# tgp-team/torch-geometric-pool

Hardware: NVIDIA B200
Metric: coarsened graphs/s (Reduce+Connect fwd+bwd) (higher is better)
Workload: dtype f32

## Files before the change

torch-geometric-pool_b200/csrc/dense_bwd_fused.cu:

```cuda
#include <stdlib.h>
#include <string.h>

#include "dense.cuh"
#include "tc_gemm.cuh"
#include "tc_ptx.cuh"

namespace tgp {
namespace tc {

extern long long* g_engine_dbg;

namespace {

#ifndef TGPB200_BWD_EPI_WARPS
#define TGPB200_BWD_EPI_WARPS 4
#endif
#ifndef TGPB200_ABL
#define TGPB200_ABL 0
#endif
#ifndef TGPB200_BWD_CONCAT
#define TGPB200_BWD_CONCAT 0
#endif
constexpr bool kConcat = TGPB200_BWD_CONCAT != 0;
constexpr int kPairs = 7;
constexpr int kGroups = 2;
constexpr int kSlots = kConcat ? 2 : 4;
static_assert(kSlots % kGroups == 0, "every operand slot must belong to ONE split group (its waiters see every phase)");
constexpr int kEpiW = TGPB200_BWD_EPI_WARPS;
constexpr int kThreadsBwd = 64 + kGroups * 128 + kEpiW * 32;
constexpr int BK = 32, KSTEPS = 4;
constexpr int BNB = 64;
constexpr uint32_t kAccW = kConcat ? 128 : 64;
constexpr uint32_t kColW = 0, kColS = kAccW, kColX = 2 * kAccW, kColRing = 2 * kAccW + 128, kRing = 64;
static_assert(kColRing + kSlots * kRing <= 512, "tensor memory budget");
constexpr uint32_t kABytes = BM * kStageRowBytes, kBBytes = BNB * kStageRowBytes;
constexpr uint32_t kStage = kABytes + 2 * kBBytes;
constexpr uint32_t kEpiBufs = kEpiW == 4 ? 2 : 1;
constexpr uint32_t kEpiBytes = kEpiW * kEpiBufs * 4096;
constexpr uint32_t kHookBytes = BM * BNB * 4;

enum ASrc { kAKMajor = 0, kAMnPlain = 1, kATmem = 2 };

struct BwdParams {
  CUtensorMap map_a[kPairs], map_b[kPairs];
  int kd[kPairs], a_src[kPairs], b_mn[kPairs], b_n0[kPairs], first[kPairs], wide[kPairs];
  uint32_t acc_col[kPairs];
  int num_pairs;
  int batch, N, K, F;
  int m_tiles, num_items, stages;
  CUtensorMap map_ds, map_dx;
  const float* S;
  const float* d;
  const float* coef;
  const float* uv;
  float eps;
  long long* dbg;
};

__global__ void __launch_bounds__(kThreadsBwd, 1) k_dense_bwd_fused(const __grid_constant__ BwdParams P) {
  extern __shared__ __align__(1024) uint8_t smem_raw[];
  uint8_t* smem = reinterpret_cast<uint8_t*>((reinterpret_cast<uintptr_t>(smem_raw) + 1023) & ~(uintptr_t)1023);
  const int stages = P.stages;
  uint64_t* bars = reinterpret_cast<uint64_t*>(smem + (size_t)kStage * stages + kEpiBytes + kHookBytes);
  const uint32_t bar_base = smem_u32(bars);
  auto bar_full = [&](int s) { return bar_base + 8u * s; };
  auto bar_lo = [&](int s) { return bar_base + 8u * (stages + s); };
  auto bar_empty = [&](int s) { return bar_base + 8u * (2 * stages + s); };
  auto bar_tfree = [&](int g) { return bar_base + 8u * (3 * stages + g); };
  const uint32_t bar_wfull = bar_base + 8u * (3 * stages + kSlots), bar_tfull = bar_wfull + 8u, bar_tempty = bar_wfull + 16u;
  uint32_t* tmem_slot = reinterpret_cast<uint32_t*>(bars + 3 * stages + kSlots + 3);

  const int warp = threadIdx.x >> 5, lane = threadIdx.x & 31;
  const uint32_t smem_base = smem_u32(smem);
  if (P.dbg && threadIdx.x == 0) {
    unsigned long long t;
    uint32_t smid;
    asm volatile("mov.u64 %0, %%globaltimer;" : "=l"(t));
    asm volatile("mov.u32 %0, %%smid;" : "=r"(smid));
    P.dbg[(200 + blockIdx.x) * 8 + 0] = (long long)t;
    P.dbg[(200 + blockIdx.x) * 8 + 2] = (long long)smid;
  }

  if (warp == 0 && lane == 0) {
    for (int s = 0; s < stages; ++s) {
      mbar_init(bar_full(s), 1);
      mbar_init(bar_lo(s), 4);
      mbar_init(bar_empty(s), 1);
    }
    for (int g = 0; g < kSlots; ++g) mbar_init(bar_tfree(g), 1);
    mbar_init(bar_wfull, 1);
    mbar_init(bar_tfull, 1);
    mbar_init(bar_tempty, kEpiW);
    fence_barrier_init();
  }
  if (warp == 1) tmem_alloc(smem_u32(tmem_slot), 512);
  tc_fence_before();
  __syncthreads();
  tc_fence_after();
  const uint32_t tmem_base = *tmem_slot;


  if (warp == 0) {
    int s = 0;
    uint32_t ph = 0;
    for (int item = blockIdx.x; item < P.num_items; item += gridDim.x) {
      const int mt = item % P.m_tiles, b = item / P.m_tiles;
      const int m0 = mt * BM;
      for (int p = 0; p < P.num_pairs; ++p) {
        const int src = P.a_src[p];
        for (int kb = 0, nkb = (P.kd[p] + BK - 1) / BK; kb < nkb; ++kb) {
          mbar_wait(bar_empty(s), ph ^ 1);
          const uint32_t sa = smem_base + (uint32_t)s * kStage, sb = sa + kABytes;
          const int k0 = kb * BK;
          if ((TGPB200_ABL & 64) && elect_one()) mbar_arrive(bar_full(s));
          if (!(TGPB200_ABL & 64) && elect_one()) {
            const bool load_a = src != kATmem && !(TGPB200_ABL & 32);
            mbar_arrive_expect_tx(bar_full(s), (load_a ? kABytes : 0u) + kBBytes);
            if (!load_a) {
            } else if (src == kAMnPlain) tma_load_3d(sa, &P.map_a[p], bar_full(s), m0, k0, b);
            else if (src == kAKMajor) tma_load_3d(sa, &P.map_a[p], bar_full(s), k0, m0, b);
            if (P.b_mn[p]) {
              for (int blk = 0; blk < BNB / 32; ++blk)
                tma_load_3d(sb + blk * (BK * kStageRowBytes), &P.map_b[p], bar_full(s), P.b_n0[p] + blk * 32, k0, b);
            } else {
              tma_load_3d(sb, &P.map_b[p], bar_full(s), k0, P.b_n0[p], b);
            }
          }
          __syncwarp();
          if (++s == stages) { s = 0; ph ^= 1; }
        }
      }
    }
  } else if (warp == 1) {
    const uint32_t tm = __shfl_sync(kFull, tmem_base, 0);
    if (elect_one()) {
      int s = 0;
      uint32_t ph = 0, kc = 0;
      int it = 0;
      for (int item = blockIdx.x; item < P.num_items; item += gridDim.x, ++it) {
        for (int p = 0; p < P.num_pairs; ++p) {
          if (p == 1) {
            mbar_wait(bar_tempty, ((uint32_t)it & 1u) ^ 1u);
            tc_fence_after();
          }
          const uint32_t d_tmem = tm + P.acc_col[p];
          const uint32_t idesc = (1u << 4) | (2u << 7) | (2u << 10) | ((uint32_t)P.b_mn[p] << 16) |
                                 ((uint32_t)(BNB >> 3) << 17) | ((uint32_t)(BM >> 4) << 24);
          const uint32_t b_lbo = P.b_mn[p] ? BK * kStageRowBytes : 16;
          const uint32_t b_step = P.b_mn[p] ? 8 * kStageRowBytes : 32;
          const uint64_t desc_b0 = make_desc(smem_base, b_lbo, P.b_mn[p] ? 512 : 1024, P.b_mn[p] ? 1 : 2);
          const uint32_t idesc2 = (idesc & ~(0x3fu << 17)) | ((uint32_t)((2 * BNB) >> 3) << 17);
          const bool wide = kConcat && P.wide[p] != 0;
          uint32_t accum = P.first[p] ? 0u : 1u;
          for (int kb = 0, nkb = (P.kd[p] + BK - 1) / BK; kb < nkb; ++kb, ++kc) {
            if (P.dbg && blockIdx.x == 0 && kc < 128) P.dbg[kc * 8 + 7] = clock64();
            mbar_wait(bar_lo(s), ph);
            if (P.dbg && blockIdx.x == 0 && kc < 128) P.dbg[kc * 8 + 5] = clock64();
            if (!(TGPB200_ABL & 1024)) tc_fence_after();
            const uint32_t ts = kc % (uint32_t)kSlots;
            const uint32_t a_stage = tm + kColRing + ts * kRing;
            const uint64_t db0 = desc_b0 + (uint64_t)(((uint32_t)s * kStage + kABytes) >> 4);
#pragma unroll
            for (int kk = 0; kk < ((TGPB200_ABL & 128) ? 0 : KSTEPS); ++kk) {
              const uint64_t db = db0 + (uint64_t)(kk * (b_step >> 4)), db_lo = db + (kBBytes >> 4);
              const uint32_t a_hi = a_stage + (uint32_t)(kk * 16), a_lo = a_hi + 8;
              if (wide) {
                umma_ts_tf32(d_tmem, a_hi, db, idesc2, kk == 0 ? accum : 1u);
                umma_ts_tf32(d_tmem, a_lo, db, idesc, 1u);
              } else {
                umma_ts_tf32(d_tmem, a_lo, db, idesc, kk == 0 ? accum : 1u);
                umma_ts_tf32(d_tmem, a_hi, db_lo, idesc, 1u);
                umma_ts_tf32(d_tmem, a_hi, db, idesc, 1u);
              }
            }
            if (P.dbg && blockIdx.x == 0 && kc < 128) P.dbg[kc * 8 + 0] = clock64();
            if (TGPB200_ABL & 4096) mbar_arrive(bar_empty(s)); else umma_commit(bar_empty(s));
            if (TGPB200_ABL & 8192) mbar_arrive(bar_tfree(ts)); else umma_commit(bar_tfree(ts));
            if (P.dbg && blockIdx.x == 0 && kc < 128) P.dbg[kc * 8 + 6] = clock64();
            accum = 1;
            if (++s == stages) { s = 0; ph ^= 1; }
          }
          if (p == 0) umma_commit(bar_wfull);
        }
        umma_commit(bar_tfull);
      }
    }
    __syncwarp();
  } else if (warp < 2 + kGroups * 4) {
    const int grp = (warp - 2) >> 2;
    const int t = (threadIdx.x - 64) & 127;
    const int q = warp & 3;
    const int m_local = q * 32 + lane;
    int s = 0;
    uint32_t ph = 0, kc = 0;
    int it = 0;
    for (int item = blockIdx.x; item < P.num_items; item += gridDim.x, ++it) {
      for (int p = 0; p < P.num_pairs; ++p) {
        const int src = P.a_src[p];
        for (int kb = 0, nkb = (P.kd[p] + BK - 1) / BK; kb < nkb; ++kb, ++kc) {
          if ((int)(kc % (uint32_t)kGroups) != grp) {
            mbar_wait(bar_full(s), ph);
            if (++s == stages) { s = 0; ph ^= 1; }
            continue;
          }
          mbar_wait(bar_full(s), ph);
          const uint32_t sa = smem_base + (uint32_t)s * kStage, sb = sa + kABytes;
          for (uint32_t ch = t; ch < ((TGPB200_ABL & 1) ? 0u : kBBytes / 16); ch += 128) {
            const float4 v = lds128(sb + ch * 16);
            float4 h, l;
            h.x = rna_tf32(v.x), h.y = rna_tf32(v.y), h.z = rna_tf32(v.z), h.w = rna_tf32(v.w);
            l.x = v.x - h.x, l.y = v.y - h.y, l.z = v.z - h.z, l.w = v.w - h.w;
            sts128(sb + ch * 16, h);
            sts128(sb + kBBytes + ch * 16, l);
          }
          if (!(TGPB200_ABL & 2)) fence_proxy_async();
          float x[32];
          if (TGPB200_ABL & 4) {
#pragma unroll
            for (int k = 0; k < 32; ++k) x[k] = (float)(k + lane);
          } else if (src == kATmem) {
            mbar_wait(bar_wfull, (uint32_t)it & 1u);
            tc_fence_after();
            tmem_ld32(tmem_base + ((uint32_t)(q * 32) << 16) + kColW + (uint32_t)(kb * BK), x);
            if (kConcat) {
              float x2[32];
              tmem_ld32(tmem_base + ((uint32_t)(q * 32) << 16) + kColW + 64u + (uint32_t)(kb * BK), x2);
#pragma unroll
              for (int k = 0; k < 32; ++k) x[k] += x2[k];
            }
          } else if (src == kAMnPlain) {
#pragma unroll
            for (int k = 0; k < 32; ++k) x[k] = lds32(sa + (uint32_t)k * (BM * 4) + (uint32_t)m_local * 4);
          } else {
#pragma unroll
            for (int c = 0; c < 8; ++c) {
              const float4 v = lds128(sa + (uint32_t)m_local * kStageRowBytes + (uint32_t)((c ^ (m_local & 7)) << 4));
              x[4 * c] = v.x, x[4 * c + 1] = v.y, x[4 * c + 2] = v.z, x[4 * c + 3] = v.w;
            }
          }
          const uint32_t slot = kc % (uint32_t)kSlots;
          if (TGPB200_ABL & 16384) {
            __syncwarp();
            if (lane == 0) mbar_arrive(bar_lo(s));
            if (++s == stages) { s = 0; ph ^= 1; }
            continue;
          }
          mbar_wait(bar_tfree(slot), ((kc / (uint32_t)kSlots) & 1u) ^ 1u);
          tc_fence_after();
          const uint32_t a_stage = tmem_base + ((uint32_t)(q * 32) << 16) + kColRing + slot * kRing;
#pragma unroll
          for (int kk = 0; kk < KSTEPS; ++kk) {
            float hi[8], lo[8];
#pragma unroll
            for (int i = 0; i < 8; ++i) {
              hi[i] = rna_tf32(x[kk * 8 + i]);
              lo[i] = x[kk * 8 + i] - hi[i];
            }
            if (!(TGPB200_ABL & 8)) tmem_st16(a_stage + (uint32_t)(kk * 16), hi, lo);
            else if (hi[0] == 123.456f && lo[7] == 3.f) P.dbg[0] = 1;
          }
          tmem_st_wait();
          tc_fence_before();
          __syncwarp();
          if (lane == 0) mbar_arrive(bar_lo(s));
          if (P.dbg && blockIdx.x == 0 && lane == 0 && kc < 128) P.dbg[kc * 8 + 1 + q] = clock64();
          if (++s == stages) { s = 0; ph ^= 1; }
        }
      }
    }
  } else {
    const int quad = warp & 3;
    const int ew = warp - 2 - kGroups * 4;
    const int e2 = ew >> 2;
    const uint32_t stg0 = smem_base + (uint32_t)kStage * stages + (uint32_t)ew * kEpiBufs * 4096u;
    uint32_t n_stored = 0;
    const uint32_t hook0 = smem_base + (uint32_t)kStage * stages + kEpiBytes;
    const int n_chunks = 2 + (P.F + 31) / 32;
    int it = 0;
    for (int item = blockIdx.x; item < P.num_items; item += gridDim.x, ++it) {
      const int mt = item % P.m_tiles, b = item / P.m_tiles;
      const int m_base = mt * BM + quad * 32;
      const int m = m_base + lane;
      float dd = 0.f, c_ent = 0.f, di = 0.f;
      bool hook = false;
      const uint32_t hrow = hook0 + (uint32_t)(quad * 32 + lane) * (BNB * 4);
      if (!(TGPB200_ABL & 256) && P.S != nullptr && m < P.N) {
        const float c_den = P.coef[b * 4 + 0];
        c_ent = P.coef[b * 4 + 2];
        hook = c_den != 0.f || c_ent != 0.f;
        if (hook) {
          dd = 2.f * c_den * P.d[(int64_t)b * P.N + m];
          const float* srow = P.S + ((int64_t)b * P.N + m) * P.K;
          for (int j = 0; j * 4 < P.K; ++j) cp_async16(hrow + (uint32_t)((j ^ (lane & 7)) << 4), srow + j * 4);
        }
        if (P.uv != nullptr) di = P.d[(int64_t)b * P.N + m];
      }
      cp_async_commit();
      mbar_wait(bar_tfull, (uint32_t)it & 1u);
      if (P.dbg && blockIdx.x == 0 && ew == 0 && lane == 0 && it < 32) P.dbg[(128 + it) * 8 + 0] = clock64();
      tc_fence_after();
      cp_async_wait_all();
      __syncwarp();
      for (int c = 0; c < ((TGPB200_ABL & 16) ? 0 : n_chunks); ++c) {
        if (kEpiW == 8 && (c & 1) != e2) continue;
        const bool is_ds = c < 2;
        const int n0 = is_ds ? c * 32 : (c - 2) * 32;
        float v[32];
        tmem_ld32(tmem_base + ((uint32_t)(quad * 32) << 16) + (is_ds ? kColS : kColX) + (uint32_t)n0, v);
        if (kConcat && is_ds) {
          float v2[32];
          tmem_ld32(tmem_base + ((uint32_t)(quad * 32) << 16) + kColS + 64u + (uint32_t)n0, v2);
#pragma unroll
          for (int j = 0; j < 32; ++j) v[j] += v2[j];
        }
        if (m_base >= P.N || n0 >= (is_ds ? P.K : P.F)) continue;
        if (is_ds && hook) {
#pragma unroll
          for (int c4 = 0; c4 < 8; ++c4) {
            if (n0 + c4 * 4 < P.K) {
              const float4 t4 = lds128(hrow + (uint32_t)((((n0 >> 2) + c4) ^ (lane & 7)) << 4));
              const float sv[4] = {t4.x, t4.y, t4.z, t4.w};
#pragma unroll
              for (int j = 0; j < 4; ++j) {
                float add = dd * sv[j];
                if (c_ent != 0.f) add += c_ent * (-__logf(sv[j] + P.eps) - __fdividef(sv[j], sv[j] + P.eps));
                v[c4 * 4 + j] += add;
              }
            }
          }
        }
        if (is_ds && P.uv != nullptr) {
          const float* ub = P.uv + (int64_t)b * 2 * P.K + n0;
#pragma unroll
          for (int j = 0; j < 32; ++j)
            if (n0 + j < P.K) v[j] += fmaf(di, __ldg(ub + j), __ldg(ub + P.K + j));
        }
        const uint32_t stg = stg0 + (n_stored % kEpiBufs) * 4096u;
        ++n_stored;
        if (lane == 0) {
          if (kEpiBufs == 2) tma_store_wait_read<1>();
          else tma_store_wait_read<0>();
        }
        __syncwarp();
        const uint32_t row = stg + (uint32_t)lane * 128u;
#pragma unroll
        for (int c4 = 0; c4 < 8; ++c4)
          sts128(row + (uint32_t)((c4 ^ (lane & 7)) << 4), make_float4(v[4 * c4], v[4 * c4 + 1], v[4 * c4 + 2], v[4 * c4 + 3]));
        fence_proxy_async();
        __syncwarp();
        if (lane == 0 && !(TGPB200_ABL & 512)) {
          tma_store_3d(is_ds ? &P.map_ds : &P.map_dx, stg, n0, m_base, b);
          tma_store_commit();
        }
      }
      tc_fence_before();
      __syncwarp();
      if (lane == 0) mbar_arrive(bar_tempty);
      if (P.dbg && blockIdx.x == 0 && ew == 0 && lane == 0 && it < 32) P.dbg[(128 + it) * 8 + 1] = clock64();
    }
    if (lane == 0) tma_store_wait_all();
  }

  tc_fence_before();
  __syncthreads();
  if (P.dbg && threadIdx.x == 0) {
    unsigned long long t;
    asm volatile("mov.u64 %0, %%globaltimer;" : "=l"(t));
    P.dbg[(200 + blockIdx.x) * 8 + 1] = (long long)t;
  }
  if (warp == 1) tmem_dealloc(tmem_base, 512);
}

bool make_out_map(CUtensorMap* map, float* ptr, int64_t batch, int64_t rows, int64_t cols) {
  EncodeTiledFn fn = encode_fn();
  if (!fn || ((uintptr_t)ptr & 15) || (cols % 4)) return false;
  cuuint64_t dims[3] = {(cuuint64_t)cols, (cuuint64_t)rows, (cuuint64_t)batch};
  cuuint64_t strides[2] = {(cuuint64_t)cols * 4, (cuuint64_t)rows * cols * 4};
  cuuint32_t box[3] = {32, 32, 1}, estr[3] = {1, 1, 1};
  return fn(map, CU_TENSOR_MAP_DATA_TYPE_FLOAT32, 3, ptr, dims, strides, box, estr, CU_TENSOR_MAP_INTERLEAVE_NONE,
            CU_TENSOR_MAP_SWIZZLE_128B, CU_TENSOR_MAP_L2_PROMOTION_NONE, CU_TENSOR_MAP_FLOAT_OOB_FILL_NONE) == CUDA_SUCCESS;
}

}

int dense_bwd_fused(const float* A, const float* S, const float* X, const float* Tt, const float* Gx, const float* Graw,
                    const float* Pm, int B, int N, int K, int F, const float* ew_S, const float* ew_d, const float* ew_coef,
                    const float* ew_uv, float eps, float* dS, float* dX, cudaStream_t stream) {
  {
    const char* e = getenv("TGPB200_BWD_FUSED");
    if (e && e[0] == '0') return TGPB200_ERR_UNSUPPORTED;
  }
  if (!A || !S || !X || !Tt || !Gx || !Graw || !dS || !dX || B <= 0) return TGPB200_ERR_UNSUPPORTED;
  if (K > BNB || F > 128 || (N % 4) || (K % 4) || (F % 4) || N < 1) return TGPB200_ERR_UNSUPPORTED;
  const uintptr_t al = (uintptr_t)A | (uintptr_t)S | (uintptr_t)X | (uintptr_t)Tt | (uintptr_t)Gx | (uintptr_t)Graw |
                       (uintptr_t)(Pm ? Pm : Graw);
  if (al & 15) return TGPB200_ERR_UNSUPPORTED;
  BwdParams P;
  memset(&P, 0, sizeof(P));
  P.batch = B, P.N = N, P.K = K, P.F = F;
  P.m_tiles = (N + BM - 1) / BM;
  P.num_items = B * P.m_tiles;
  const int64_t NN = (int64_t)N * N, NK = (int64_t)N * K, NF = (int64_t)N * F, KK = (int64_t)K * K, KF = (int64_t)K * F;
  int n = 0;
  bool ok = true;
  auto add = [&](int kd, int a_src, OperandDesc a, OperandDesc b, int b_n0, uint32_t acc, int first) {
    P.kd[n] = kd, P.a_src[n] = a_src, P.b_mn[n] = b.mn_major, P.b_n0[n] = b_n0, P.acc_col[n] = acc, P.first[n] = first;
    P.wide[n] = acc != kColX && acc != kColX + (uint32_t)BNB;
    if (a_src == kAKMajor) ok = ok && make_operand_map(&P.map_a[n], a, false, B, N, kd, BM);
    else if (a_src == kAMnPlain) ok = ok && make_operand_map_mn_plain(&P.map_a[n], a, B, N, kd);
    ok = ok && make_operand_map(&P.map_b[n], b, false, B, b.mn_major ? (int)b.row_stride : (int)(b.batch_stride / b.row_stride), kd, BNB);
    ++n;
  };
  add(N, kAKMajor, OperandDesc{A, NN, N, 0}, OperandDesc{S, NK, K, 1}, 0, kColW, 1);
  add(F, kAKMajor, OperandDesc{X, NF, F, 0}, OperandDesc{Gx, KF, F, 0}, 0, kColS, 1);
  add(K, kAMnPlain, OperandDesc{Tt, NK, N, 1}, OperandDesc{Graw, KK, K, 1}, 0, kColS, 0);
  if (Pm) add(K, kAKMajor, OperandDesc{S, NK, K, 0}, OperandDesc{Pm, KK, K, 1}, 0, kColS, 0);
  add(K, kATmem, OperandDesc{nullptr, 0, 0, 0}, OperandDesc{Graw, KK, K, 0}, 0, kColS, 0);
  for (int j = 0; j * BNB < F; ++j)
    add(K, kAKMajor, OperandDesc{S, NK, K, 0}, OperandDesc{Gx, KF, F, 1}, j * BNB, kColX + (uint32_t)(j * BNB), 1);
  if (!ok) return TGPB200_ERR_UNSUPPORTED;
  P.num_pairs = n;
  if (!make_out_map(&P.map_ds, dS, B, N, K) || !make_out_map(&P.map_dx, dX, B, N, F)) return TGPB200_ERR_UNSUPPORTED;
  P.S = ew_S, P.d = ew_d, P.coef = ew_coef, P.uv = ew_S ? ew_uv : nullptr, P.eps = eps;
  P.stages = 5;
  {
    const char* e = getenv("TGPB200_BWD_STAGES");
    if (e && atoi(e) >= 2 && atoi(e) <= 5) P.stages = atoi(e);
  }
  P.dbg = g_engine_dbg;
  static bool attr_set = false;
  if (!attr_set) {
    attr_set = true;
    cudaFuncSetAttribute(k_dense_bwd_fused, cudaFuncAttributeMaxDynamicSharedMemorySize, 227 * 1024);
  }
  const size_t smem = (size_t)kStage * P.stages + kEpiBytes + kHookBytes + (3 * P.stages + kSlots + 4) * 8 + 16 + 1024;
  const int sms = device_sm_count();
  const int grid = P.num_items < sms ? P.num_items : sms;
  launch("k_dense_bwd_fused", k_dense_bwd_fused, grid, kThreadsBwd, smem, stream, P);
  return launch_status();
}

}
}
```

torch-geometric-pool_b200/csrc/tc_ptx.cuh:

```cuda
#pragma once
#include <cuda.h>
#include <stdio.h>

#include "common.cuh"

namespace tgp {
namespace tc {

__device__ __forceinline__ uint32_t smem_u32(const void* p) { return (uint32_t)__cvta_generic_to_shared(p); }

__device__ __forceinline__ void mbar_init(uint32_t bar, uint32_t count) {
  asm volatile("mbarrier.init.shared::cta.b64 [%0], %1;" ::"r"(bar), "r"(count));
}
__device__ __forceinline__ void mbar_arrive(uint32_t bar) {
  asm volatile("mbarrier.arrive.shared::cta.b64 _, [%0];" ::"r"(bar) : "memory");
}
__device__ __forceinline__ void mbar_arrive_expect_tx(uint32_t bar, uint32_t bytes) {
  asm volatile("mbarrier.arrive.expect_tx.shared::cta.b64 _, [%0], %1;" ::"r"(bar), "r"(bytes) : "memory");
}
__device__ __forceinline__ void mbar_wait(uint32_t bar, uint32_t parity) {
  uint32_t done = 0;
  uint64_t spins = 0;
  while (true) {
    asm volatile(
        "{\n"
        ".reg .pred p;\n"
        "mbarrier.try_wait.parity.shared::cta.b64 p, [%1], %2;\n"
        "selp.u32 %0, 1, 0, p;\n"
        "}\n"
        : "=r"(done)
        : "r"(bar), "r"(parity)
        : "memory");
    if (done) break;
    if (++spins > (1ull << 26)) {
      printf("[tgp_b200] mbarrier wait timed out (block %d thread %d bar %u parity %u)\n", blockIdx.x, threadIdx.x, bar,
             parity);
      __trap();
    }
  }
}
__device__ __forceinline__ bool elect_one() {
  uint32_t pred;
  asm volatile("{\n.reg .pred p;\nelect.sync _|p, 0xffffffff;\nselp.u32 %0, 1, 0, p;\n}\n" : "=r"(pred));
  return pred != 0;
}
__device__ __forceinline__ void fence_barrier_init() { asm volatile("fence.mbarrier_init.release.cluster;" ::: "memory"); }
__device__ __forceinline__ void fence_proxy_async() { asm volatile("fence.proxy.async.shared::cta;" ::: "memory"); }
__device__ __forceinline__ void tc_fence_before() { asm volatile("tcgen05.fence::before_thread_sync;" ::: "memory"); }
__device__ __forceinline__ void tc_fence_after() { asm volatile("tcgen05.fence::after_thread_sync;" ::: "memory"); }

__device__ __forceinline__ void tma_load_3d(uint32_t dst, const CUtensorMap* map, uint32_t bar, int c0, int c1, int c2) {
  asm volatile(
      "cp.async.bulk.tensor.3d.shared::cluster.global.mbarrier::complete_tx::bytes [%0], [%1, {%3, %4, %5}], [%2];" ::"r"(dst),
      "l"(map), "r"(bar), "r"(c0), "r"(c1), "r"(c2)
      : "memory");
}
__device__ __forceinline__ void tma_load_4d(uint32_t dst, const CUtensorMap* map, uint32_t bar, int c0, int c1, int c2,
                                            int c3) {
  asm volatile(
      "cp.async.bulk.tensor.4d.shared::cluster.global.mbarrier::complete_tx::bytes [%0], [%1, {%3, %4, %5, %6}], [%2];" ::"r"(
          dst),
      "l"(map), "r"(bar), "r"(c0), "r"(c1), "r"(c2), "r"(c3)
      : "memory");
}

__device__ __forceinline__ void tma_store_3d(const CUtensorMap* map, uint32_t src, int c0, int c1, int c2) {
  asm volatile("cp.async.bulk.tensor.3d.global.shared::cta.bulk_group [%0, {%2, %3, %4}], [%1];" ::"l"(map), "r"(src),
               "r"(c0), "r"(c1), "r"(c2)
               : "memory");
}
__device__ __forceinline__ void tma_store_commit() { asm volatile("cp.async.bulk.commit_group;" ::: "memory"); }
template <int kPending>
__device__ __forceinline__ void tma_store_wait_read() {
  asm volatile("cp.async.bulk.wait_group.read %0;" ::"n"(kPending) : "memory");
}
__device__ __forceinline__ void tma_store_wait_all() { asm volatile("cp.async.bulk.wait_group 0;" ::: "memory"); }
__device__ __forceinline__ void cp_async16(uint32_t dst, const void* src) {
  asm volatile("cp.async.cg.shared.global [%0], [%1], 16;" ::"r"(dst), "l"(src) : "memory");
}
__device__ __forceinline__ void cp_async_commit() { asm volatile("cp.async.commit_group;" ::: "memory"); }
__device__ __forceinline__ void cp_async_wait_all() { asm volatile("cp.async.wait_group 0;" ::: "memory"); }
__device__ __forceinline__ void sts32(uint32_t addr, uint32_t v) {
  asm volatile("st.shared.u32 [%0], %1;" ::"r"(addr), "r"(v) : "memory");
}
__device__ __forceinline__ void sts128u(uint32_t addr, const uint4& v) {
  asm volatile("st.shared.v4.u32 [%0], {%1, %2, %3, %4};" ::"r"(addr), "r"(v.x), "r"(v.y), "r"(v.z), "r"(v.w) : "memory");
}

__device__ __forceinline__ void tmem_alloc(uint32_t dst_smem, uint32_t ncols) {
  asm volatile("tcgen05.alloc.cta_group::1.sync.aligned.shared::cta.b32 [%0], %1;" ::"r"(dst_smem), "r"(ncols) : "memory");
  asm volatile("tcgen05.relinquish_alloc_permit.cta_group::1.sync.aligned;" ::: "memory");
}
__device__ __forceinline__ void tmem_dealloc(uint32_t addr, uint32_t ncols) {
  asm volatile("tcgen05.dealloc.cta_group::1.sync.aligned.b32 %0, %1;" ::"r"(addr), "r"(ncols) : "memory");
}
__device__ __forceinline__ void umma_commit(uint32_t bar) {
  asm volatile("tcgen05.commit.cta_group::1.mbarrier::arrive::one.shared::cluster.b64 [%0];" ::"r"(bar) : "memory");
}
template <bool kTf32>
__device__ __forceinline__ void umma(uint32_t tmem_d, uint64_t desc_a, uint64_t desc_b, uint32_t idesc, uint32_t accum) {
  if (kTf32) {
    asm volatile(
        "{\n.reg .pred p;\nsetp.ne.b32 p, %4, 0;\n"
        "tcgen05.mma.cta_group::1.kind::tf32 [%0], %1, %2, %3, p;\n}\n" ::"r"(tmem_d),
        "l"(desc_a), "l"(desc_b), "r"(idesc), "r"(accum)
        : "memory");
  } else {
    asm volatile(
        "{\n.reg .pred p;\nsetp.ne.b32 p, %4, 0;\n"
        "tcgen05.mma.cta_group::1.kind::f16 [%0], %1, %2, %3, p;\n}\n" ::"r"(tmem_d),
        "l"(desc_a), "l"(desc_b), "r"(idesc), "r"(accum)
        : "memory");
  }
}
__device__ __forceinline__ uint32_t cluster_ctarank() {
  uint32_t r;
  asm volatile("mov.u32 %0, %%cluster_ctarank;" : "=r"(r));
  return r;
}
__device__ __forceinline__ uint32_t mapa_shared(uint32_t addr, uint32_t rank) {
  uint32_t r;
  asm volatile("mapa.shared::cluster.u32 %0, %1, %2;" : "=r"(r) : "r"(addr), "r"(rank));
  return r;
}
__device__ __forceinline__ void cluster_sync_all() {
  asm volatile("barrier.cluster.arrive.release.aligned;" ::: "memory");
  asm volatile("barrier.cluster.wait.acquire.aligned;" ::: "memory");
}
__device__ __forceinline__ void mbar_arrive_cluster(uint32_t cluster_bar) {
  asm volatile("mbarrier.arrive.release.cluster.shared::cluster.b64 _, [%0];" ::"r"(cluster_bar) : "memory");
}
__device__ __forceinline__ void tma_load_3d_pair(uint32_t dst, const CUtensorMap* map, uint32_t leader_bar, int c0, int c1,
                                                 int c2) {
  asm volatile(
      "cp.async.bulk.tensor.3d.cta_group::2.shared::cluster.global.mbarrier::complete_tx::bytes [%0], [%1, {%3, %4, %5}], [%2];" ::
          "r"(dst),
      "l"(map), "r"(leader_bar), "r"(c0), "r"(c1), "r"(c2)
      : "memory");
}
__device__ __forceinline__ void tmem_alloc_pair(uint32_t dst_smem, uint32_t ncols) {
  asm volatile("tcgen05.alloc.cta_group::2.sync.aligned.shared::cta.b32 [%0], %1;" ::"r"(dst_smem), "r"(ncols) : "memory");
  asm volatile("tcgen05.relinquish_alloc_permit.cta_group::2.sync.aligned;" ::: "memory");
}
__device__ __forceinline__ void tmem_dealloc_pair(uint32_t addr, uint32_t ncols) {
  asm volatile("tcgen05.dealloc.cta_group::2.sync.aligned.b32 %0, %1;" ::"r"(addr), "r"(ncols) : "memory");
}
__device__ __forceinline__ void umma_commit_pair(uint32_t bar) {
  asm volatile(
      "{\n.reg .b16 m;\nmov.b16 m, 3;\n"
      "tcgen05.commit.cta_group::2.mbarrier::arrive::one.shared::cluster.multicast::cluster.b64 [%0], m;\n}\n" ::"r"(bar)
      : "memory");
}
__device__ __forceinline__ void umma_pair_bf16(uint32_t tmem_d, uint64_t desc_a, uint64_t desc_b, uint32_t idesc,
                                               uint32_t accum) {
  asm volatile(
      "{\n.reg .pred p;\nsetp.ne.b32 p, %4, 0;\n"
      "tcgen05.mma.cta_group::2.kind::f16 [%0], %1, %2, %3, p;\n}\n" ::"r"(tmem_d),
      "l"(desc_a), "l"(desc_b), "r"(idesc), "r"(accum)
      : "memory");
}

__device__ __forceinline__ void tmem_ld32(uint32_t taddr, float (&v)[32]) {
  uint32_t r[32];
  asm volatile(
      "tcgen05.ld.sync.aligned.32x32b.x32.b32 "
      "{%0, %1, %2, %3, %4, %5, %6, %7, %8, %9, %10, %11, %12, %13, %14, %15, "
      "%16, %17, %18, %19, %20, %21, %22, %23, %24, %25, %26, %27, %28, %29, %30, %31}, [%32];"
      : "=r"(r[0]), "=r"(r[1]), "=r"(r[2]), "=r"(r[3]), "=r"(r[4]), "=r"(r[5]), "=r"(r[6]), "=r"(r[7]), "=r"(r[8]),
        "=r"(r[9]), "=r"(r[10]), "=r"(r[11]), "=r"(r[12]), "=r"(r[13]), "=r"(r[14]), "=r"(r[15]), "=r"(r[16]),
        "=r"(r[17]), "=r"(r[18]), "=r"(r[19]), "=r"(r[20]), "=r"(r[21]), "=r"(r[22]), "=r"(r[23]), "=r"(r[24]),
        "=r"(r[25]), "=r"(r[26]), "=r"(r[27]), "=r"(r[28]), "=r"(r[29]), "=r"(r[30]), "=r"(r[31])
      : "r"(taddr));
  asm volatile("tcgen05.wait::ld.sync.aligned;" ::: "memory");
#pragma unroll
  for (int i = 0; i < 32; ++i) v[i] = __uint_as_float(r[i]);
}

__device__ __forceinline__ float rna_tf32(float x) {
  return __uint_as_float((__float_as_uint(x) + 0x1000u) & 0xffffe000u);
}

__device__ __forceinline__ float4 lds128(uint32_t addr) {
  float4 v;
  asm volatile("ld.shared.v4.f32 {%0, %1, %2, %3}, [%4];" : "=f"(v.x), "=f"(v.y), "=f"(v.z), "=f"(v.w) : "r"(addr));
  return v;
}
__device__ __forceinline__ void sts128(uint32_t addr, const float4& v) {
  asm volatile("st.shared.v4.f32 [%0], {%1, %2, %3, %4};" ::"r"(addr), "f"(v.x), "f"(v.y), "f"(v.z), "f"(v.w) : "memory");
}
__device__ __forceinline__ uint4 lds128u(uint32_t addr) {
  uint4 v;
  asm volatile("ld.shared.v4.u32 {%0, %1, %2, %3}, [%4];" : "=r"(v.x), "=r"(v.y), "=r"(v.z), "=r"(v.w) : "r"(addr));
  return v;
}

__device__ __forceinline__ float lds32(uint32_t addr) {
  float v;
  asm volatile("ld.shared.f32 %0, [%1];" : "=f"(v) : "r"(addr));
  return v;
}
__device__ __forceinline__ void tmem_st16(uint32_t taddr, const float (&a)[8], const float (&b)[8]) {
  asm volatile(
      "tcgen05.st.sync.aligned.32x32b.x16.b32 [%0], "
      "{%1, %2, %3, %4, %5, %6, %7, %8, %9, %10, %11, %12, %13, %14, %15, %16};" ::"r"(taddr),
      "r"(__float_as_uint(a[0])), "r"(__float_as_uint(a[1])), "r"(__float_as_uint(a[2])), "r"(__float_as_uint(a[3])),
      "r"(__float_as_uint(a[4])), "r"(__float_as_uint(a[5])), "r"(__float_as_uint(a[6])), "r"(__float_as_uint(a[7])),
      "r"(__float_as_uint(b[0])), "r"(__float_as_uint(b[1])), "r"(__float_as_uint(b[2])), "r"(__float_as_uint(b[3])),
      "r"(__float_as_uint(b[4])), "r"(__float_as_uint(b[5])), "r"(__float_as_uint(b[6])), "r"(__float_as_uint(b[7]))
      : "memory");
}
__device__ __forceinline__ void tmem_st_wait() { asm volatile("tcgen05.wait::st.sync.aligned;" ::: "memory"); }
__device__ __forceinline__ void umma_ts_tf32(uint32_t tmem_d, uint32_t tmem_a, uint64_t desc_b, uint32_t idesc,
                                             uint32_t accum) {
  asm volatile(
      "{\n.reg .pred p;\nsetp.ne.b32 p, %4, 0;\n"
      "tcgen05.mma.cta_group::1.kind::tf32 [%0], [%1], %2, %3, p;\n}\n" ::"r"(tmem_d),
      "r"(tmem_a), "l"(desc_b), "r"(idesc), "r"(accum)
      : "memory");
}

__device__ __forceinline__ uint64_t make_desc(uint32_t saddr, uint32_t lbo_bytes, uint32_t sbo_bytes,
                                              uint32_t layout_type = 2) {
  uint64_t d = 0;
  d |= (uint64_t)((saddr >> 4) & 0x3fff);
  d |= (uint64_t)((lbo_bytes >> 4) & 0x3fff) << 16;
  d |= (uint64_t)((sbo_bytes >> 4) & 0x3fff) << 32;
  d |= (uint64_t)1 << 46;
  d |= (uint64_t)layout_type << 61;
  return d;
}


}
}
```

Baseline: 2.251 million.

## Template backward fused kernel on k-block size and default to two-atom BK=64

The backward fused 3xTF32 kernel is templated on the k-block size. The default is now 64, two swizzle atoms per pipeline stage, which halves the number of barrier round-trips and commits per pair. To fit shared memory, the B lo split is now written over the raw A tile instead of a separate buffer. The A-operand hi/lo split into the tensor-memory ring now runs in 16-column chunks before the B split, and stage count is derived from the shared-memory budget. Larger stages may lower the stage count, and the reordering adds an extra named barrier per group.

Result: no change. 2.254 million, median of 6 (+0.2%).

```diff
diff --git a/torch-geometric-pool_b200/csrc/dense_bwd_fused.cu b/torch-geometric-pool_b200/csrc/dense_bwd_fused.cu
--- a/torch-geometric-pool_b200/csrc/dense_bwd_fused.cu
+++ b/torch-geometric-pool_b200/csrc/dense_bwd_fused.cu
@@ -24,27 +24,36 @@
 constexpr bool kConcat = TGPB200_BWD_CONCAT != 0;
 constexpr int kPairs = 7;
 constexpr int kGroups = 2;
-constexpr int kSlots = kConcat ? 2 : 4;
-static_assert(kSlots % kGroups == 0, "every operand slot must belong to ONE split group (its waiters see every phase)");
 constexpr int kEpiW = TGPB200_BWD_EPI_WARPS;
 constexpr int kThreadsBwd = 64 + kGroups * 128 + kEpiW * 32;
-constexpr int BK = 32, KSTEPS = 4;
 constexpr int BNB = 64;
-constexpr uint32_t kAccW = kConcat ? 128 : 64;
-constexpr uint32_t kColW = 0, kColS = kAccW, kColX = 2 * kAccW, kColRing = 2 * kAccW + 128, kRing = 64;
-static_assert(kColRing + kSlots * kRing <= 512, "tensor memory budget");
-constexpr uint32_t kABytes = BM * kStageRowBytes, kBBytes = BNB * kStageRowBytes;
-constexpr uint32_t kStage = kABytes + 2 * kBBytes;
+constexpr int kAtomK = 32, kAtomSteps = 4;
+constexpr uint32_t kAAtom = BM * kStageRowBytes, kBAtom = BNB * kStageRowBytes;
 constexpr uint32_t kEpiBufs = kEpiW == 4 ? 2 : 1;
 constexpr uint32_t kEpiBytes = kEpiW * kEpiBufs * 4096;
 constexpr uint32_t kHookBytes = BM * BNB * 4;
 
+template <int kBK>
+struct BwdCfg {
+  static constexpr int kAtoms = kBK / kAtomK;
+  static constexpr bool kCat = kConcat && kBK == 32;
+  static constexpr int kSlots = (kCat || kBK == 64) ? 2 : 4;
+  static constexpr uint32_t kAccW = kCat ? 128 : 64;
+  static constexpr uint32_t kColW = 0, kColS = kAccW, kColX = 2 * kAccW, kColRing = 2 * kAccW + 128, kRing = 2 * kBK;
+  static constexpr uint32_t kABytes = kAtoms * kAAtom, kBBytes = kAtoms * kBAtom;
+  static constexpr uint32_t kStage = kABytes + kBBytes;
+  static_assert(kBBytes <= kABytes, "B lo is written over the raw A tile");
+  static_assert(kBK == 32 || kBK == 64, "k-block of one or two swizzle atoms");
+  static_assert(kColRing + kSlots * kRing <= 512, "tensor memory budget");
+  static_assert(kSlots % kGroups == 0, "every operand slot must belong to ONE split group (its waiters see every phase)");
+};
+
 enum ASrc { kAKMajor = 0, kAMnPlain = 1, kATmem = 2 };
+enum Acc { kAccWId = 0, kAccSId = 1, kAccXId = 2 };
 
 struct BwdParams {
   CUtensorMap map_a[kPairs], map_b[kPairs];
-  int kd[kPairs], a_src[kPairs], b_mn[kPairs], b_n0[kPairs], first[kPairs], wide[kPairs];
-  uint32_t acc_col[kPairs];
+  int kd[kPairs], a_src[kPairs], b_mn[kPairs], b_n0[kPairs], first[kPairs], acc[kPairs];
   int num_pairs;
   int batch, N, K, F;
   int m_tiles, num_items, stages;
@@ -57,7 +66,17 @@
   long long* dbg;
 };
 
+template <int kBK>
+__device__ __forceinline__ int atoms_in(int kd, int k0) {
+  const int n = (kd - k0 + kAtomK - 1) / kAtomK;
+  return n < BwdCfg<kBK>::kAtoms ? n : BwdCfg<kBK>::kAtoms;
+}
+
+template <int kBK>
 __global__ void __launch_bounds__(kThreadsBwd, 1) k_dense_bwd_fused(const __grid_constant__ BwdParams P) {
+  using C = BwdCfg<kBK>;
+  constexpr int kSlots = C::kSlots;
+  constexpr uint32_t kStage = C::kStage, kABytes = C::kABytes, kBBytes = C::kBBytes;
   extern __shared__ __align__(1024) uint8_t smem_raw[];
   uint8_t* smem = reinterpret_cast<uint8_t*>((reinterpret_cast<uintptr_t>(smem_raw) + 1023) & ~(uintptr_t)1023);
   const int stages = P.stages;
@@ -108,22 +127,26 @@
       const int m0 = mt * BM;
       for (int p = 0; p < P.num_pairs; ++p) {
         const int src = P.a_src[p];
-        for (int kb = 0, nkb = (P.kd[p] + BK - 1) / BK; kb < nkb; ++kb) {
+        for (int kb = 0, nkb = (P.kd[p] + kBK - 1) / kBK; kb < nkb; ++kb) {
           mbar_wait(bar_empty(s), ph ^ 1);
           const uint32_t sa = smem_base + (uint32_t)s * kStage, sb = sa + kABytes;
-          const int k0 = kb * BK;
+          const int k0 = kb * kBK, na = atoms_in<kBK>(P.kd[p], k0);
           if ((TGPB200_ABL & 64) && elect_one()) mbar_arrive(bar_full(s));
           if (!(TGPB200_ABL & 64) && elect_one()) {
             const bool load_a = src != kATmem && !(TGPB200_ABL & 32);
-            mbar_arrive_expect_tx(bar_full(s), (load_a ? kABytes : 0u) + kBBytes);
-            if (!load_a) {
-            } else if (src == kAMnPlain) tma_load_3d(sa, &P.map_a[p], bar_full(s), m0, k0, b);
-            else if (src == kAKMajor) tma_load_3d(sa, &P.map_a[p], bar_full(s), k0, m0, b);
-            if (P.b_mn[p]) {
-              for (int blk = 0; blk < BNB / 32; ++blk)
-                tma_load_3d(sb + blk * (BK * kStageRowBytes), &P.map_b[p], bar_full(s), P.b_n0[p] + blk * 32, k0, b);
-            } else {
-              tma_load_3d(sb, &P.map_b[p], bar_full(s), k0, P.b_n0[p], b);
+            mbar_arrive_expect_tx(bar_full(s), (uint32_t)na * ((load_a ? kAAtom : 0u) + kBAtom));
+            for (int h = 0; h < na; ++h) {
+              const int kh = k0 + h * kAtomK;
+              const uint32_t ah = sa + (uint32_t)h * kAAtom, bh = sb + (uint32_t)h * kBAtom;
+              if (!load_a) {
+              } else if (src == kAMnPlain) tma_load_3d(ah, &P.map_a[p], bar_full(s), m0, kh, b);
+              else if (src == kAKMajor) tma_load_3d(ah, &P.map_a[p], bar_full(s), kh, m0, b);
+              if (P.b_mn[p]) {
+                for (int blk = 0; blk < BNB / 32; ++blk)
+                  tma_load_3d(bh + blk * (kAtomK * kStageRowBytes), &P.map_b[p], bar_full(s), P.b_n0[p] + blk * 32, kh, b);
+              } else {
+                tma_load_3d(bh, &P.map_b[p], bar_full(s), kh, P.b_n0[p], b);
+              }
             }
           }
           __syncwarp();
@@ -143,34 +166,42 @@
             mbar_wait(bar_tempty, ((uint32_t)it & 1u) ^ 1u);
             tc_fence_after();
           }
-          const uint32_t d_tmem = tm + P.acc_col[p];
+          const int acc = P.acc[p];
+          const uint32_t d_tmem =
+              tm + (acc == kAccWId ? C::kColW : acc == kAccSId ? C::kColS : C::kColX + (uint32_t)((acc - kAccXId) * BNB));
           const uint32_t idesc = (1u << 4) | (2u << 7) | (2u << 10) | ((uint32_t)P.b_mn[p] << 16) |
                                  ((uint32_t)(BNB >> 3) << 17) | ((uint32_t)(BM >> 4) << 24);
-          const uint32_t b_lbo = P.b_mn[p] ? BK * kStageRowBytes : 16;
+          const uint32_t b_lbo = P.b_mn[p] ? kAtomK * kStageRowBytes : 16;
           const uint32_t b_step = P.b_mn[p] ? 8 * kStageRowBytes : 32;
           const uint64_t desc_b0 = make_desc(smem_base, b_lbo, P.b_mn[p] ? 512 : 1024, P.b_mn[p] ? 1 : 2);
           const uint32_t idesc2 = (idesc & ~(0x3fu << 17)) | ((uint32_t)((2 * BNB) >> 3) << 17);
-          const bool wide = kConcat && P.wide[p] != 0;
+          const bool wide = C::kCat && acc < kAccXId;
           uint32_t accum = P.first[p] ? 0u : 1u;
-          for (int kb = 0, nkb = (P.kd[p] + BK - 1) / BK; kb < nkb; ++kb, ++kc) {
+          for (int kb = 0, nkb = (P.kd[p] + kBK - 1) / kBK; kb < nkb; ++kb, ++kc) {
+            const int na = atoms_in<kBK>(P.kd[p], kb * kBK);
             if (P.dbg && blockIdx.x == 0 && kc < 128) P.dbg[kc * 8 + 7] = clock64();
             mbar_wait(bar_lo(s), ph);
             if (P.dbg && blockIdx.x == 0 && kc < 128) P.dbg[kc * 8 + 5] = clock64();
             if (!(TGPB200_ABL & 1024)) tc_fence_after();
             const uint32_t ts = kc % (uint32_t)kSlots;
-            const uint32_t a_stage = tm + kColRing + ts * kRing;
+            const uint32_t a_stage = tm + C::kColRing + ts * C::kRing;
             const uint64_t db0 = desc_b0 + (uint64_t)(((uint32_t)s * kStage + kABytes) >> 4);
 #pragma unroll
-            for (int kk = 0; kk < ((TGPB200_ABL & 128) ? 0 : KSTEPS); ++kk) {
-              const uint64_t db = db0 + (uint64_t)(kk * (b_step >> 4)), db_lo = db + (kBBytes >> 4);
-              const uint32_t a_hi = a_stage + (uint32_t)(kk * 16), a_lo = a_hi + 8;
-              if (wide) {
-                umma_ts_tf32(d_tmem, a_hi, db, idesc2, kk == 0 ? accum : 1u);
-                umma_ts_tf32(d_tmem, a_lo, db, idesc, 1u);
-              } else {
-                umma_ts_tf32(d_tmem, a_lo, db, idesc, kk == 0 ? accum : 1u);
-                umma_ts_tf32(d_tmem, a_hi, db_lo, idesc, 1u);
-                umma_ts_tf32(d_tmem, a_hi, db, idesc, 1u);
+            for (int h = 0; h < C::kAtoms; ++h) {
+              if (h >= na) break;
+#pragma unroll
+              for (int j = 0; j < ((TGPB200_ABL & 128) ? 0 : kAtomSteps); ++j) {
+                const int kk = h * kAtomSteps + j;
+                const uint64_t db = db0 + (uint64_t)((h * kBAtom + j * b_step) >> 4), db_lo = db - (kABytes >> 4);
+                const uint32_t a_hi = a_stage + (uint32_t)(kk * 16), a_lo = a_hi + 8;
+                if (wide) {
+                  umma_ts_tf32(d_tmem, a_hi, db, idesc2, kk == 0 ? accum : 1u);
+                  umma_ts_tf32(d_tmem, a_lo, db, idesc, 1u);
+                } else {
+                  umma_ts_tf32(d_tmem, a_lo, db, idesc, kk == 0 ? accum : 1u);
+                  umma_ts_tf32(d_tmem, a_hi, db_lo, idesc, 1u);
+                  umma_ts_tf32(d_tmem, a_hi, db, idesc, 1u);
+                }
               }
             }
             if (P.dbg && blockIdx.x == 0 && kc < 128) P.dbg[kc * 8 + 0] = clock64();
@@ -197,70 +228,83 @@
     for (int item = blockIdx.x; item < P.num_items; item += gridDim.x, ++it) {
       for (int p = 0; p < P.num_pairs; ++p) {
         const int src = P.a_src[p];
-        for (int kb = 0, nkb = (P.kd[p] + BK - 1) / BK; kb < nkb; ++kb, ++kc) {
+        for (int kb = 0, nkb = (P.kd[p] + kBK - 1) / kBK; kb < nkb; ++kb, ++kc) {
           if ((int)(kc % (uint32_t)kGroups) != grp) {
             mbar_wait(bar_full(s), ph);
             if (++s == stages) { s = 0; ph ^= 1; }
             continue;
           }
           mbar_wait(bar_full(s), ph);
+          const int na = atoms_in<kBK>(P.kd[p], kb * kBK);
           const uint32_t sa = smem_base + (uint32_t)s * kStage, sb = sa + kABytes;
+          const bool skeleton = TGPB200_ABL & 16384;
+          if (!skeleton) {
+            if (src == kATmem) {
+              mbar_wait(bar_wfull, (uint32_t)it & 1u);
+              tc_fence_after();
+            }
+            const uint32_t slot = kc % (uint32_t)kSlots;
+            const uint32_t a_ring = tmem_base + ((uint32_t)(q * 32) << 16) + C::kColRing + slot * C::kRing;
+#pragma unroll
+            for (int g = 0; g < 2 * C::kAtoms; ++g) {
+              if (g >= 2 * na) break;
+              const uint32_t ah = sa + (uint32_t)(g >> 1) * kAAtom;
+              float x[16];
+              if (TGPB200_ABL & 4) {
+#pragma unroll
+                for (int k = 0; k < 16; ++k) x[k] = (float)(k + lane);
+              } else if (src == kATmem) {
+                const uint32_t wcol = C::kColW + (uint32_t)(kb * kBK + g * 16);
+                tmem_ld16(tmem_base + ((uint32_t)(q * 32) << 16) + wcol, x);
+                if (C::kCat) {
+                  float x2[16];
+                  tmem_ld16(tmem_base + ((uint32_t)(q * 32) << 16) + wcol + 64u, x2);
+#pragma unroll
+                  for (int k = 0; k < 16; ++k) x[k] += x2[k];
+                }
+              } else if (src == kAMnPlain) {
+#pragma unroll
+                for (int k = 0; k < 16; ++k)
+                  x[k] = lds32(ah + (uint32_t)((g & 1) * 16 + k) * (BM * 4) + (uint32_t)m_local * 4);
+              } else {
+#pragma unroll
+                for (int c = 0; c < 4; ++c) {
+                  const int cc = (g & 1) * 4 + c;
+                  const float4 v = lds128(ah + (uint32_t)m_local * kStageRowBytes + (uint32_t)((cc ^ (m_local & 7)) << 4));
+                  x[4 * c] = v.x, x[4 * c + 1] = v.y, x[4 * c + 2] = v.z, x[4 * c + 3] = v.w;
+                }
+              }
+              if (g == 0) {
+                mbar_wait(bar_tfree(slot), ((kc / (uint32_t)kSlots) & 1u) ^ 1u);
+                tc_fence_after();
+              }
+#pragma unroll
+              for (int kk = 0; kk < 2; ++kk) {
+                float hi[8], lo[8];
+#pragma unroll
+                for (int i = 0; i < 8; ++i) {
+                  hi[i] = rna_tf32(x[kk * 8 + i]);
+                  lo[i] = x[kk * 8 + i] - hi[i];
+                }
+                if (!(TGPB200_ABL & 8)) tmem_st16(a_ring + (uint32_t)((2 * g + kk) * 16), hi, lo);
+                else if (hi[0] == 123.456f && lo[7] == 3.f) P.dbg[0] = 1;
+              }
+            }
+            asm volatile("bar.sync %0, 128;" ::"r"(1 + grp) : "memory");
+          }
           for (uint32_t ch = t; ch < ((TGPB200_ABL & 1) ? 0u : kBBytes / 16); ch += 128) {
             const float4 v = lds128(sb + ch * 16);
             float4 h, l;
             h.x = rna_tf32(v.x), h.y = rna_tf32(v.y), h.z = rna_tf32(v.z), h.w = rna_tf32(v.w);
             l.x = v.x - h.x, l.y = v.y - h.y, l.z = v.z - h.z, l.w = v.w - h.w;
             sts128(sb + ch * 16, h);
-            sts128(sb + kBBytes + ch * 16, l);
+            sts128(sa + ch * 16, l);
           }
           if (!(TGPB200_ABL & 2)) fence_proxy_async();
-          float x[32];
-          if (TGPB200_ABL & 4) {
-#pragma unroll
-            for (int k = 0; k < 32; ++k) x[k] = (float)(k + lane);
-          } else if (src == kATmem) {
-            mbar_wait(bar_wfull, (uint32_t)it & 1u);
-            tc_fence_after();
-            tmem_ld32(tmem_base + ((uint32_t)(q * 32) << 16) + kColW + (uint32_t)(kb * BK), x);
-            if (kConcat) {
-              float x2[32];
-              tmem_ld32(tmem_base + ((uint32_t)(q * 32) << 16) + kColW + 64u + (uint32_t)(kb * BK), x2);
-#pragma unroll
-              for (int k = 0; k < 32; ++k) x[k] += x2[k];
-            }
-          } else if (src == kAMnPlain) {
-#pragma unroll
-            for (int k = 0; k < 32; ++k) x[k] = lds32(sa + (uint32_t)k * (BM * 4) + (uint32_t)m_local * 4);
-          } else {
-#pragma unroll
-            for (int c = 0; c < 8; ++c) {
-              const float4 v = lds128(sa + (uint32_t)m_local * kStageRowBytes + (uint32_t)((c ^ (m_local & 7)) << 4));
-              x[4 * c] = v.x, x[4 * c + 1] = v.y, x[4 * c + 2] = v.z, x[4 * c + 3] = v.w;
-            }
-          }
-          const uint32_t slot = kc % (uint32_t)kSlots;
-          if (TGPB200_ABL & 16384) {
-            __syncwarp();
-            if (lane == 0) mbar_arrive(bar_lo(s));
-            if (++s == stages) { s = 0; ph ^= 1; }
-            continue;
-          }
-          mbar_wait(bar_tfree(slot), ((kc / (uint32_t)kSlots) & 1u) ^ 1u);
-          tc_fence_after();
-          const uint32_t a_stage = tmem_base + ((uint32_t)(q * 32) << 16) + kColRing + slot * kRing;
-#pragma unroll
-          for (int kk = 0; kk < KSTEPS; ++kk) {
-            float hi[8], lo[8];
-#pragma unroll
-            for (int i = 0; i < 8; ++i) {
-              hi[i] = rna_tf32(x[kk * 8 + i]);
-              lo[i] = x[kk * 8 + i] - hi[i];
-            }
-            if (!(TGPB200_ABL & 8)) tmem_st16(a_stage + (uint32_t)(kk * 16), hi, lo);
-            else if (hi[0] == 123.456f && lo[7] == 3.f) P.dbg[0] = 1;
-          }
-          tmem_st_wait();
-          tc_fence_before();
+          if (!skeleton) {
+            tmem_st_wait();
+            tc_fence_before();
+          }
           __syncwarp();
           if (lane == 0) mbar_arrive(bar_lo(s));
           if (P.dbg && blockIdx.x == 0 && lane == 0 && kc < 128) P.dbg[kc * 8 + 1 + q] = clock64();
@@ -306,10 +350,10 @@
         const bool is_ds = c < 2;
         const int n0 = is_ds ? c * 32 : (c - 2) * 32;
         float v[32];
-        tmem_ld32(tmem_base + ((uint32_t)(quad * 32) << 16) + (is_ds ? kColS : kColX) + (uint32_t)n0, v);
-        if (kConcat && is_ds) {
+        tmem_ld32(tmem_base + ((uint32_t)(quad * 32) << 16) + (is_ds ? C::kColS : C::kColX) + (uint32_t)n0, v);
+        if (C::kCat && is_ds) {
           float v2[32];
-          tmem_ld32(tmem_base + ((uint32_t)(quad * 32) << 16) + kColS + 64u + (uint32_t)n0, v2);
+          tmem_ld32(tmem_base + ((uint32_t)(quad * 32) << 16) + C::kColS + 64u + (uint32_t)n0, v2);
 #pragma unroll
           for (int j = 0; j < 32; ++j) v[j] += v2[j];
         }
@@ -369,6 +413,30 @@
     P.dbg[(200 + blockIdx.x) * 8 + 1] = (long long)t;
   }
   if (warp == 1) tmem_dealloc(tmem_base, 512);
+}
+
+template <int kBK>
+int launch_bwd(BwdParams& P, const char* name, cudaStream_t stream) {
+  using C = BwdCfg<kBK>;
+  auto smem_for = [](int stages) {
+    return (size_t)C::kStage * stages + kEpiBytes + kHookBytes + (3 * stages + C::kSlots + 4) * 8 + 16 + 1024;
+  };
+  int max_stages = 5;
+  while (max_stages > 2 && smem_for(max_stages) > 227 * 1024) --max_stages;
+  P.stages = max_stages;
+  {
+    const char* e = getenv("TGPB200_BWD_STAGES");
+    if (e && atoi(e) >= 2 && atoi(e) <= max_stages) P.stages = atoi(e);
+  }
+  static bool attr_set = false;
+  if (!attr_set) {
+    attr_set = true;
+    cudaFuncSetAttribute(k_dense_bwd_fused<kBK>, cudaFuncAttributeMaxDynamicSharedMemorySize, 227 * 1024);
+  }
+  const int sms = device_sm_count();
+  const int grid = P.num_items < sms ? P.num_items : sms;
+  launch(name, k_dense_bwd_fused<kBK>, grid, kThreadsBwd, smem_for(P.stages), stream, P);
+  return launch_status();
 }
 
 bool make_out_map(CUtensorMap* map, float* ptr, int64_t batch, int64_t rows, int64_t cols) {
@@ -403,42 +471,31 @@
   const int64_t NN = (int64_t)N * N, NK = (int64_t)N * K, NF = (int64_t)N * F, KK = (int64_t)K * K, KF = (int64_t)K * F;
   int n = 0;
   bool ok = true;
-  auto add = [&](int kd, int a_src, OperandDesc a, OperandDesc b, int b_n0, uint32_t acc, int first) {
-    P.kd[n] = kd, P.a_src[n] = a_src, P.b_mn[n] = b.mn_major, P.b_n0[n] = b_n0, P.acc_col[n] = acc, P.first[n] = first;
-    P.wide[n] = acc != kColX && acc != kColX + (uint32_t)BNB;
+  auto add = [&](int kd, int a_src, OperandDesc a, OperandDesc b, int b_n0, int acc, int first) {
+    P.kd[n] = kd, P.a_src[n] = a_src, P.b_mn[n] = b.mn_major, P.b_n0[n] = b_n0, P.acc[n] = acc, P.first[n] = first;
     if (a_src == kAKMajor) ok = ok && make_operand_map(&P.map_a[n], a, false, B, N, kd, BM);
     else if (a_src == kAMnPlain) ok = ok && make_operand_map_mn_plain(&P.map_a[n], a, B, N, kd);
     ok = ok && make_operand_map(&P.map_b[n], b, false, B, b.mn_major ? (int)b.row_stride : (int)(b.batch_stride / b.row_stride), kd, BNB);
     ++n;
   };
-  add(N, kAKMajor, OperandDesc{A, NN, N, 0}, OperandDesc{S, NK, K, 1}, 0, kColW, 1);
-  add(F, kAKMajor, OperandDesc{X, NF, F, 0}, OperandDesc{Gx, KF, F, 0}, 0, kColS, 1);
-  add(K, kAMnPlain, OperandDesc{Tt, NK, N, 1}, OperandDesc{Graw, KK, K, 1}, 0, kColS, 0);
-  if (Pm) add(K, kAKMajor, OperandDesc{S, NK, K, 0}, OperandDesc{Pm, KK, K, 1}, 0, kColS, 0);
-  add(K, kATmem, OperandDesc{nullptr, 0, 0, 0}, OperandDesc{Graw, KK, K, 0}, 0, kColS, 0);
+  add(N, kAKMajor, OperandDesc{A, NN, N, 0}, OperandDesc{S, NK, K, 1}, 0, kAccWId, 1);
+  add(F, kAKMajor, OperandDesc{X, NF, F, 0}, OperandDesc{Gx, KF, F, 0}, 0, kAccSId, 1);
+  add(K, kAMnPlain, OperandDesc{Tt, NK, N, 1}, OperandDesc{Graw, KK, K, 1}, 0, kAccSId, 0);
+  if (Pm) add(K, kAKMajor, OperandDesc{S, NK, K, 0}, OperandDesc{Pm, KK, K, 1}, 0, kAccSId, 0);
+  add(K, kATmem, OperandDesc{nullptr, 0, 0, 0}, OperandDesc{Graw, KK, K, 0}, 0, kAccSId, 0);
   for (int j = 0; j * BNB < F; ++j)
-    add(K, kAKMajor, OperandDesc{S, NK, K, 0}, OperandDesc{Gx, KF, F, 1}, j * BNB, kColX + (uint32_t)(j * BNB), 1);
+    add(K, kAKMajor, OperandDesc{S, NK, K, 0}, OperandDesc{Gx, KF, F, 1}, j * BNB, kAccXId + j, 1);
   if (!ok) return TGPB200_ERR_UNSUPPORTED;
   P.num_pairs = n;
   if (!make_out_map(&P.map_ds, dS, B, N, K) || !make_out_map(&P.map_dx, dX, B, N, F)) return TGPB200_ERR_UNSUPPORTED;
   P.S = ew_S, P.d = ew_d, P.coef = ew_coef, P.uv = ew_S ? ew_uv : nullptr, P.eps = eps;
-  P.stages = 5;
+  P.dbg = g_engine_dbg;
   {
-    const char* e = getenv("TGPB200_BWD_STAGES");
-    if (e && atoi(e) >= 2 && atoi(e) <= 5) P.stages = atoi(e);
-  }
-  P.dbg = g_engine_dbg;
-  static bool attr_set = false;
-  if (!attr_set) {
-    attr_set = true;
-    cudaFuncSetAttribute(k_dense_bwd_fused, cudaFuncAttributeMaxDynamicSharedMemorySize, 227 * 1024);
-  }
-  const size_t smem = (size_t)kStage * P.stages + kEpiBytes + kHookBytes + (3 * P.stages + kSlots + 4) * 8 + 16 + 1024;
-  const int sms = device_sm_count();
-  const int grid = P.num_items < sms ? P.num_items : sms;
-  launch("k_dense_bwd_fused", k_dense_bwd_fused, grid, kThreadsBwd, smem, stream, P);
-  return launch_status();
-}
-
-}
-}
+    const char* e = getenv("TGPB200_BWD_BK");
+    if (e && atoi(e) == 32) return launch_bwd<32>(P, "k_dense_bwd_fused_bk32", stream);
+  }
+  return launch_bwd<64>(P, "k_dense_bwd_fused", stream);
+}
+
+}
+}
diff --git a/torch-geometric-pool_b200/csrc/tc_ptx.cuh b/torch-geometric-pool_b200/csrc/tc_ptx.cuh
--- a/torch-geometric-pool_b200/csrc/tc_ptx.cuh
+++ b/torch-geometric-pool_b200/csrc/tc_ptx.cuh
@@ -176,6 +176,19 @@
   for (int i = 0; i < 32; ++i) v[i] = __uint_as_float(r[i]);
 }
 
+__device__ __forceinline__ void tmem_ld16(uint32_t taddr, float (&v)[16]) {
+  uint32_t r[16];
+  asm volatile(
+      "tcgen05.ld.sync.aligned.32x32b.x16.b32 "
+      "{%0, %1, %2, %3, %4, %5, %6, %7, %8, %9, %10, %11, %12, %13, %14, %15}, [%16];"
+      : "=r"(r[0]), "=r"(r[1]), "=r"(r[2]), "=r"(r[3]), "=r"(r[4]), "=r"(r[5]), "=r"(r[6]), "=r"(r[7]), "=r"(r[8]),
+        "=r"(r[9]), "=r"(r[10]), "=r"(r[11]), "=r"(r[12]), "=r"(r[13]), "=r"(r[14]), "=r"(r[15])
+      : "r"(taddr));
+  asm volatile("tcgen05.wait::ld.sync.aligned;" ::: "memory");
+#pragma unroll
+  for (int i = 0; i < 16; ++i) v[i] = __uint_as_float(r[i]);
+}
+
 __device__ __forceinline__ float rna_tf32(float x) {
   return __uint_as_float((__float_as_uint(x) + 0x1000u) & 0xffffe000u);
 }
```
